# wadx2019/rpo

Measured on AMD Instinct MI355X. Metric: env-steps/sec (whole node), SafeCartpole-v0 (CartSafe-v0) RPODDPG, rollout + one batch-256 constrained policy update per vector step, higher is better.
Workload: dtype f32; 1 GPU; CartSafe-v0 RPODDPG, 4096 vectorised envs per MI355X, scripts/cart_exp.py hyper-parameters, update batch 256 every vector step (reference cadence), replay capacity 20000 per env; envs_per_gpu=4096, global_envs=4096, update_batch=256, hip_graph=True, training_batch_projection=row-wise, rccl_ranks=0, collectives_in_graph=False, graphs_replayed_on_all_ranks=True, graph_capture_fell_back_to_eager=False

## Files before the change

### rpo_amd/csrc/fused.hip

```cpp
#include <stdlib.h>

#include <type_traits>

#include "cartsafe_dev.h"
#include "heads_dev.h"
#include "mlp_bwd.h"
#include "mlp_tile.h"
#include "pendulum_dev.h"
#include "rollout_args.h"
#include "rollout_env.h"

namespace {

using namespace rpo_mlp_dev;
using rpo_cart_dev::ActArgs;
using rpo_cart_dev::CartConsts;
using rpo_cart_dev::cart_explore_project;
using rpo_cart_dev::load_consts;

Mlp to_dev(const rpo_mlp* h) {
    return Mlp{h->Ws, h->bs, h->Wa, h->ba, h->W0, h->b0, h->W1, h->b1, h->W1b, h->b1b, h->S, h->A, h->E, h->H, h->n_out, h->cat, h->head_dim};
}


#ifndef RPO_ROLLOUT_SKIP
#define RPO_ROLLOUT_SKIP 0
#endif

template <class ENV, int EIN, int H, int RT>
__global__ __launch_bounds__(kFwdThreads) void rollout_kernel(RolloutArgs<ENV> p, typename ENV::Consts c) {
    typedef TileLds<EIN, RT, 8, 8> Lds;
    __shared__ Lds lds;
    constexpr int kInS = Lds::kS;
    constexpr int kLanes = rpo_mlp_dev::kRows * RT;
    constexpr int kStats = 10;
    const int row0 = blockIdx.x * kLanes;
    const int tid = threadIdx.x;
    const int n = p.step.n;
    const long long t = p.step.ctrl ? p.step.ctrl[RPO_CTRL_T] : 0;
    RpoEpisode ep{0, 0.0f, 0u};
    if (tid < kLanes && row0 + tid < n) ep = ENV::episode(p.step, row0 + tid);
    ENV::stage_obs(p.step, row0, kLanes, lds.in_s, kInS);
    float draw = 0.0f;
    const bool philox_noise = !p.gauss && p.act.noise_mode == RPO_NOISE_PHILOX;
    if (!(RPO_ROLLOUT_SKIP & 8) && tid < kLanes && row0 + tid < n && (p.gauss || philox_noise)) {
        const rpo_u4 u = p.gauss ? rpo_philox(p.act.seed, p.act.env_id_base + (uint32_t)(row0 + tid), (uint32_t)t, RPO_STREAM_POLICY,
                                              (uint32_t)p.step.ctrl[RPO_CTRL_UPDATES])
                                 : rpo_philox(p.act.seed, p.act.env_id_base + (uint32_t)(row0 + tid), (uint32_t)t, RPO_STREAM_ACT);
        draw = rpo_normal(u.x, u.y);
    }
    if (RPO_ROLLOUT_SKIP & 1) {
        if (tid < 2 * kLanes) lds.out[tid] = 0.25f;
        __syncthreads();
    } else {
        mlp_tile_forward<EIN, H, RT, Lds>(p.actor, lds, row0, n, nullptr, nullptr, p.gauss ? 0 : 1, p.scale, p.base);
    }

    float st[kStats];
#pragma unroll
    for (int k = 0; k < kStats; ++k) st[k] = 0.0f;
    float iters_f = 0.0f;
    const int i = row0 + tid;
    if (tid < kLanes && i < n) {
        const float eps_t = fmaxf(p.act.eps_end, p.act.eps_start - p.act.eps_decay * (float)t);
        float ap = lds.out[tid * 2];
        if (p.gauss) {
            ap = rpo_head_dev::gauss_head_row(ap, lds.out[tid * 2 + 1], draw, p.scale, p.base, p.act.box_lo, p.act.box_hi, 0, nullptr);
        }
        int k;
        typename ENV::ActArgs act = p.act;
        if (philox_noise) {
            ap = rpo_explore_clip(ap, eps_t, draw, p.act.box_lo, p.act.box_hi);
            act.noise_mode = RPO_NOISE_NONE;
        }
        float2 a;
        if (RPO_ROLLOUT_SKIP & 2) { a = make_float2(ap, 0.5f * ap); k = 0; }
        else a = ENV::project(act, c, lds.in_s + tid * kInS, i, ap, eps_t, t, k);
        iters_f = (float)k;
        reinterpret_cast<float2*>(p.act.action)[i] = a;
        const long long ring_base = p.step.rows ? (t % p.step.cap_steps) * (long long)n : 0;
        if (!(RPO_ROLLOUT_SKIP & 4)) ENV::lane(p.step, c, i, lds.in_s + tid * kInS, a, ep, ring_base, st);
    }
    if (RPO_ROLLOUT_SKIP & 16) return;
    if (p.step.stats && tid < 64) {
        float* srow = rpo_stats_row(p.step.stats, p.step.stats_cap, t);
        const int slot[kStats + 1] = {RPO_STAT_REWARD_SUM, RPO_STAT_EPISODES, RPO_STAT_RETURN_SUM, RPO_STAT_LENGTH_SUM,
                                      RPO_STAT_MAX_INEQ_SUM, RPO_STAT_MAX_EQ_SUM, RPO_STAT_VIOL_COUNT, RPO_STAT_TERMINATED,
                                      RPO_STAT_MAX_INEQ_MAX, RPO_STAT_MAX_EQ_MAX, RPO_STAT_PROJ_ITERS};
        float red[kStats + 1];
#pragma unroll
        for (int k = 0; k < kStats; ++k) red[k] = st[k];
        red[kStats] = iters_f;
        if (kLanes <= 16) rpo_row16_reduce_many(red, 3u << 8);
        else rpo_wave_reduce_many<kStats + 1, 32>(red, 3u << 8);
        rpo_stats_commit(red, 3u << 8, slot, srow);
    }
    if (!p.defer_clock) rpo_step_epilogue(p.step.ctrl, t, p.step.stats, p.step.stats_cap);
}

template <class ENV>
int launch_rollout(const RolloutArgs<ENV>& args, const typename ENV::Consts& c, int n_envs, void* stream) {
    {
        const int sel = rpo_tune(RPO_TUNE_ROLLOUT_WIDE);
        if (sel == 3 || sel == 4 || (sel == 2 && n_envs >= RPO_ROLLOUT_STREAM_FROM)) {
            const int e = rpo_rollout_stream_launch(std::is_same<ENV, CartEnv>::value ? 0 : 1, &args, &c, n_envs, stream);
            if (e >= 0) return e;
        }
    }
    const int wide_sel = rpo_tune(RPO_TUNE_ROLLOUT_WIDE);
    const int E = args.actor.E;
    const bool wide = E == 128 && (wide_sel == 0 || wide_sel == 1 ? wide_sel != 0 : n_envs >= 64 * 192);
    if (E == 128 && wide) {
        hipLaunchKernelGGL((rollout_kernel<ENV, 128, 256, 4>), dim3((n_envs + 63) / 64), dim3(kFwdThreads), 0,
                           (hipStream_t)stream, args, c);
    } else if (E == 128) {
        hipLaunchKernelGGL((rollout_kernel<ENV, 128, 256, 1>), dim3((n_envs + 15) / 16), dim3(kFwdThreads), 0,
                           (hipStream_t)stream, args, c);
    } else if (E == 256) {
        hipLaunchKernelGGL((rollout_kernel<ENV, 256, 256, 1>), dim3((n_envs + 15) / 16), dim3(kFwdThreads), 0,
                           (hipStream_t)stream, args, c);
    } else {
        return RPO_ERR_ARG;
    }
    RPO_LAUNCH_CHECK();
    return 0;
}

int check_actor(const Mlp& actor, int obs_dim, int gauss) {
    if (actor.hd > 1 || actor.S != obs_dim || actor.A != 0 || actor.n_out != (gauss ? 2 : 1) || actor.cat || actor.H != 256 || !actor.Ws ||
        !actor.W0 || !actor.W1 || (gauss && !actor.W1b))
        return RPO_ERR_ARG;
    return 0;
}
// ... 1057 lines not shown
```

### rpo_amd/csrc/mlp_tile.h

```cpp
#pragma once
#include "common.h"

namespace rpo_mlp_dev {

typedef float f32x4 __attribute__((ext_vector_type(4)));

constexpr int kRows = 16;
constexpr int kThreads = 256;
constexpr int kFwdWaves = 8;
constexpr int kFwdThreads = kFwdWaves * 64;
constexpr int kInS = 64, kInA = 48;

struct Mlp {
    const float *Ws, *bs, *Wa, *ba, *W0, *b0, *W1, *b1, *W1b, *b1b;
    int S, A, E, H, n_out, cat;
    int hd;
    int l1_vec;
};
struct MlpGrad {
    float *Ws, *bs, *Wa, *ba, *W0, *b0, *W1, *b1, *W1b, *b1b;
};

__device__ __forceinline__ f32x4 mfma4(float a, float b, f32x4 c) {
    return __builtin_amdgcn_mfma_f32_16x16x4f32(a, b, c, 0, 0, 0);
}

template <int EIN, int RT = 1, int INS = kInS, int INA = kInA>
struct TileLds {
    static constexpr int ROWS = kRows * RT;
    static constexpr int kS = INS, kA = INA;
    __attribute__((aligned(16))) float x1[ROWS * (EIN + 4)];
    float in_s[ROWS * INS];
    float in_a[ROWS * INA];
    float part[kFwdWaves * ROWS * 2];
    float out[ROWS * 2];
};

constexpr int kWideOut = 32;

template <int EIN, int H>
struct TileLdsWide : TileLds<EIN, 1, kInS, kInA> {
    __attribute__((aligned(16))) float hr[kRows * (H + 4)];
    float outw[kRows * kWideOut];
};

template <int EIN, int H, int RT>
struct TileWeights {
    static constexpr int NT = H / (16 * kFwdWaves);
    static constexpr int ITS = EIN / 16;
    static constexpr int PRE_MAX = RT > 1 ? 4 : 16;
    static constexpr int PRE = ITS < PRE_MAX ? ITS : PRE_MAX;
    static constexpr int TPW = EIN / (16 * kFwdWaves);
    float bias;
    float ws0[8], wa0[8];
    float wk[TPW][3];
    float4 wpre[PRE][NT];
    float b0v[NT], w1av[NT], w1bv[NT];
    float b1v;
};

template <int EIN>
__device__ __forceinline__ bool tile_l1_mfma(const Mlp& net) {
    return EIN == 128 && !net.cat && net.S <= 6 && net.A <= 4 && net.S > 0 && !net.l1_vec;
}

#ifndef RPO_TILE_SKIP
#define RPO_TILE_SKIP 0
#endif

template <int EIN, int H, int RT>
__device__ __forceinline__ void tile_load_weights(const Mlp& net, TileWeights<EIN, H, RT>& w) {
    constexpr int ROWS = kRows * RT;
    constexpr int NT = TileWeights<EIN, H, RT>::NT, PRE = TileWeights<EIN, H, RT>::PRE;
    const int tid = threadIdx.x, lane = tid & 63, wave = tid >> 6;
    const int li = lane & 15, lg = lane >> 4;
    if (RPO_TILE_SKIP & 1) {
        w.bias = 0.01f * (float)li;
#pragma unroll
        for (int u = 0; u < 8; ++u) { w.ws0[u] = 0.1f; w.wa0[u] = 0.1f; }
#pragma unroll
        for (int it = 0; it < PRE; ++it)
#pragma unroll
            for (int c = 0; c < NT; ++c) w.wpre[it][c] = make_float4(0.01f, -0.01f, 0.02f, 0.01f * (float)lg);
#pragma unroll
        for (int c = 0; c < NT; ++c) { w.b0v[c] = 0.1f; w.w1av[c] = 0.05f; w.w1bv[c] = 0.0f; }
        w.b1v = 0.0f;
        return;
    }
    if (tile_l1_mfma<EIN>(net)) {
        constexpr int TPW = TileWeights<EIN, H, RT>::TPW;
        const bool add_a = net.A > 0;
        w.bias = 0.0f;
#pragma unroll
        for (int t = 0; t < TPW; ++t) {
            const int e = (wave + t * kFwdWaves) * 16 + li;
            const float* p0 = lg == 0 ? net.bs + e : (lg == 1 ? net.ba + e : net.Ws + e * net.S + (lg - 2));
            const bool live0 = lg == 0 || (lg == 1 ? add_a : lg - 2 < net.S);
            w.wk[t][0] = live0 ? *p0 : 0.0f;
            w.wk[t][1] = 2 + lg < net.S ? net.Ws[e * net.S + 2 + lg] : 0.0f;
            w.wk[t][2] = (add_a && lg < net.A) ? net.Wa[e * net.A + lg] : 0.0f;
        }
    } else {
        const int e_col = tid % EIN;
        const bool act_part = net.cat && e_col >= net.E;
        const int er = act_part ? e_col - net.E : e_col;
        const bool use_s = !act_part, use_a = net.A > 0 && (act_part || !net.cat);
        w.bias = act_part ? net.ba[er] : (net.bs[er] + ((net.A > 0 && !net.cat) ? net.ba[er] : 0.0f));
#pragma unroll
        for (int u = 0; u < 8; ++u) {
            w.ws0[u] = (use_s && u < net.S) ? net.Ws[er * net.S + u] : 0.0f;
            w.wa0[u] = (use_a && u < net.A) ? net.Wa[er * net.A + u] : 0.0f;
        }
    }
    const int j0 = wave * (H / kFwdWaves);
#pragma unroll
    for (int it = 0; it < PRE; ++it)
#pragma unroll
        for (int c = 0; c < NT; ++c)
            w.wpre[it][c] = *reinterpret_cast<const float4*>(&net.W0[(size_t)(j0 + c * 16 + li) * EIN + it * 16 + lg * 4]);
#pragma unroll
    for (int c = 0; c < NT; ++c) {
        w.b0v[c] = net.b0[j0 + c * 16 + li];
        w.w1av[c] = net.hd > 1 ? 0.0f : net.W1[j0 + c * 16 + li];
        w.w1bv[c] = (net.n_out > 1 && net.hd <= 1) ? net.W1b[j0 + c * 16 + li] : 0.0f;
    }
    w.b1v = (net.hd <= 1 && tid < ROWS * net.n_out) ? (((tid % net.n_out) == 0) ? net.b1[0] : net.b1b[0]) : 0.0f;
}

template <int EIN, int H, int RT, class LDS, bool WIDE = false>
__device__ __forceinline__ void tile_compute(const Mlp& net, const TileWeights<EIN, H, RT>& w, LDS& lds, int row0, int n,
                                             float* x0_save, float* h1_save, int out_mode, float scale, float base) {
    constexpr int kInS = LDS::kS, kInA = LDS::kA;
    constexpr int ROWS = kRows * RT;
    constexpr int LDX = EIN + 4;
    constexpr int GROUPS = kFwdThreads / EIN;
    constexpr int RPT = ROWS / GROUPS;
    static_assert(kFwdThreads % EIN == 0 && ROWS % GROUPS == 0, "layer-1 thread mapping");
    constexpr int NT = TileWeights<EIN, H, RT>::NT, ITS = TileWeights<EIN, H, RT>::ITS, PRE = TileWeights<EIN, H, RT>::PRE;
    float* x1 = lds.x1;
    const float* in_s = lds.in_s;
    const float* in_a = lds.in_a;
    float* part = lds.part;
    const int tid = threadIdx.x, lane = tid & 63, wave = tid >> 6;
    const int li = lane & 15, lg = lane >> 4;
    const int e_col = tid % EIN, r_lo = (tid / EIN) * RPT;
    const bool act_part = net.cat && e_col >= net.E;
    const int er = act_part ? e_col - net.E : e_col;
    const bool use_s = !act_part, use_a = net.A > 0 && (act_part || !net.cat);
    const int j0 = wave * (H / kFwdWaves);
    float acc1[RPT];
#pragma unroll
    for (int r = 0; r < RPT; ++r) acc1[r] = w.bias;
    __syncthreads();
    const bool l1_mfma = tile_l1_mfma<EIN>(net);
    if (l1_mfma) {
        constexpr int TPW = TileWeights<EIN, H, RT>::TPW;
        const bool x0_vec = (reinterpret_cast<uintptr_t>(x0_save) & 15u) == 0;
#pragma unroll
        for (int rt = 0; rt < RT; ++rt) {
            const int row = rt * kRows + li;
            const float b0 = lg < 2 ? 1.0f : (lg - 2 < net.S ? in_s[row * kInS + lg - 2] : 0.0f);
            const float b1 = 2 + lg < net.S ? in_s[row * kInS + 2 + lg] : 0.0f;
            const float b2 = (net.A > 0 && lg < net.A) ? in_a[row * kInA + lg] : 0.0f;
#pragma unroll
            for (int t = 0; t < TPW; ++t) {
                f32x4 c = f32x4{0.0f, 0.0f, 0.0f, 0.0f};
                if (!(RPO_TILE_SKIP & 2)) {
                    c = mfma4(w.wk[t][0], b0, c);
                    c = mfma4(w.wk[t][1], b1, c);
                    c = mfma4(w.wk[t][2], b2, c);
                }
                const int e0 = (wave + t * kFwdWaves) * 16 + 4 * lg;
                if (x0_save && row0 + row < n) {
                    float* dst = x0_save + (size_t)(row0 + row) * EIN + e0;
                    if (x0_vec) *reinterpret_cast<f32x4*>(dst) = c;
                    else { dst[0] = c[0]; dst[1] = c[1]; dst[2] = c[2]; dst[3] = c[3]; }
                }
                *reinterpret_cast<f32x4*>(&x1[row * LDX + e0]) =
                    f32x4{fmaxf(c[0], 0.0f), fmaxf(c[1], 0.0f), fmaxf(c[2], 0.0f), fmaxf(c[3], 0.0f)};
            }
        }
    }

    if (!l1_mfma && use_s && !(RPO_TILE_SKIP & 2)) {
        for (int i0 = 0; i0 < net.S; i0 += 8) {
            float wv[8];
#pragma unroll
            for (int u = 0; u < 8; ++u) wv[u] = (i0 == 0) ? w.ws0[u] : ((i0 + u < net.S) ? net.Ws[er * net.S + i0 + u] : 0.0f);
#pragma unroll
            for (int u = 0; u < 8; ++u) {
                if (i0 + u < net.S) {
#pragma unroll
                    for (int r = 0; r < RPT; ++r) acc1[r] = fmaf(in_s[(r_lo + r) * kInS + i0 + u], wv[u], acc1[r]);
                }
            }
        }
    }
    if (!l1_mfma && use_a && !(RPO_TILE_SKIP & 2)) {
        for (int i0 = 0; i0 < net.A; i0 += 8) {
            float wv[8];
#pragma unroll
            for (int u = 0; u < 8; ++u) wv[u] = (i0 == 0) ? w.wa0[u] : ((i0 + u < net.A) ? net.Wa[er * net.A + i0 + u] : 0.0f);
#pragma unroll
            for (int u = 0; u < 8; ++u) {
                if (i0 + u < net.A) {
#pragma unroll
                    for (int r = 0; r < RPT; ++r) acc1[r] = fmaf(in_a[(r_lo + r) * kInA + i0 + u], wv[u], acc1[r]);
// ... 131 lines not shown
```

### rpo_amd/csrc/nsplit.hip

```cpp
#include <stdlib.h>

#include "cartsafe_dev.h"
#include "heads_dev.h"
#include "mlp_bwd.h"
#include "nsplit_dev.h"
#include "pendulum_dev.h"
#include "rollout_env.h"

namespace {

using namespace rpo_mlp_dev;

Mlp to_dev(const rpo_mlp* h) {
    return Mlp{h->Ws, h->bs, h->Wa, h->ba, h->W0, h->b0, h->W1, h->b1, h->W1b, h->b1b, h->S, h->A, h->E, h->H, h->n_out, h->cat, h->head_dim};
}

bool split_ok(const Mlp& m) {
    return m.E == 128 && m.H == 256 && !m.cat && m.hd <= 1 && m.S <= 6 && m.A <= 4 && m.n_out >= 1 && m.n_out <= 2 && m.Ws && m.W0 &&
           m.W1 && (m.A == 0 || m.Wa) && (m.n_out == 1 || m.W1b);
}

struct NsBlock { int tile, g; };
__device__ __forceinline__ NsBlock ns_block() {
    const int lin = (int)blockIdx.x + (int)gridDim.x * (int)blockIdx.y, T = (int)gridDim.y;
// ... 724 lines not shown
        __syncthreads();
        float s0 = 0.0f, s1 = 0.0f;
        for (int b2 = tid; b2 < B; b2 += kThreads) {
            s0 += dglob[(size_t)b2 * dstride];
            if (two) s1 += dglob[(size_t)b2 * dstride + 1];
        }
        { float ss[2] = {s0, s1}; rpo_wave_reduce_many(ss, 0u); s0 = ss[0]; s1 = ss[1]; }
        float* red = smem + 256;
        if ((tid & 63) == 0) { red[(tid >> 6) * 2] = s0; red[(tid >> 6) * 2 + 1] = s1; }
        __syncthreads();
        if (tid == 0) {
            const float nb1 = cur_b1 + (((red[0] + red[2]) + red[4]) + red[6]);
            gr.b1[0] = nb1;
            gmax = fmaxf(gmax, fabsf(nb1));
            if (two) {
                const float nb1b = cur_b1b + (((red[1] + red[3]) + red[5]) + red[7]);
                gr.b1b[0] = nb1b;
                gmax = fmaxf(gmax, fabsf(nb1b));
            }
        }
    }
    return gmax;
}

__device__ __forceinline__ float ns_weight_role(const Mlp& net, const MlpGrad& gr, const float* h1, const float* x0,
                                                const float* dglob, int dstride, bool two, int B, int w, float* smem) {
    if (w < kW0Tiles) return ns_dw0_tile(net, gr.W0, h1, x0, dglob, dstride, two, B, w, smem);
    return ns_hv_block(net, gr, h1, dglob, dstride, two, B, w - kW0Tiles, smem);
}

constexpr int kBwdASmem = kRows * (256 + 4) + 16 + 4 * 16 * 16;

template <class L>
__device__ __forceinline__ void bwd_a_role(const SplitArgs& p, float* smem, int b, unsigned fused_consumers = 0u,
                                           unsigned fused_need = 0u, unsigned fused_need_critics = 0u) {
    constexpr int EIN = 128, H = 256, LDH = H + 4;
    const int T = (p.B + kRows - 1) / kRows, B = p.B;
    const int tid = threadIdx.x, lane = tid & 63, wave = tid >> 6, li = lane & 15, lg = lane >> 4;
    {
        const int k = b / (T * kNsGroups), rem = b - k * T * kNsGroups, g = rem / T, tile = rem - g * T;
        const int row0 = tile * kRows;
        const Mlp& net = p.critic[k];
        float* dh_s = smem;
        float* dq_s = smem + kRows * LDH;
        float* wpart = dq_s + 16;
        const int jw = wave * (H / 4), e = g * 16 + li;
        float wv[H / 16], hv[kRows];
#pragma unroll
        for (int ks = 0; ks < H / 16; ++ks) wv[ks] = net.W0[(size_t)(jw + ks * 4 + lg) * EIN + e];
        const float w1a = net.W1[tid];
        if (fused_consumers && fused_need_critics)
            ns_tile_wait(p.tile_sync + (T + tile) * kNsSyncStride, fused_need_critics, p.tile_sync + 3 * T * kNsSyncStride, 16);
#pragma unroll
        for (int r = 0; r < kRows; ++r) hv[r] = row0 + r < B ? p.h1[k][(size_t)(row0 + r) * H + tid] : 0.0f;
        const size_t xo = (size_t)(row0 + (tid >> 4)) * EIN + g * 16 + (tid & 15);
        const float x0v = row0 + (tid >> 4) < B ? p.x0[k][xo] : 0.0f;
        if (fused_consumers) {
            ns_tile_wait(p.tile_sync + (T + tile) * kNsSyncStride, fused_need, p.tile_sync + 3 * T * kNsSyncStride);
            ns_tile_passed(p.tile_sync, T, tile, fused_consumers);
        }
        if (tid < 64) {
            float dq = 0.0f, hub = 0.0f;
            if (tid < kRows && row0 + tid < B) {
                dq = ns_td_row<L>(p, k, row0 + tid, &hub);
                if (g == 0) p.dq[k][row0 + tid] = dq;
            }
            if (tid < kRows) dq_s[tid] = dq;
            const float sum = rpo_row16_sum_desc_lane0(hub);
            if (tid == 0 && g == 0) p.loss_partial[k * T + tile] = sum;
        }
        __syncthreads();
#pragma unroll
        for (int r = 0; r < kRows; ++r) dh_s[r * LDH + tid] = (hv[r] > 0.0f) ? dq_s[r] * w1a : 0.0f;
        __syncthreads();
        f32x4 acc = f32x4{0.0f, 0.0f, 0.0f, 0.0f};
#pragma unroll
        for (int ks = 0; ks < H / 16; ++ks) acc = mfma4(dh_s[li * LDH + jw + ks * 4 + lg], wv[ks], acc);
#pragma unroll
        for (int i = 0; i < 4; ++i) wpart[(wave * 16 + lg * 4 + i) * 16 + li] = acc[i];
        __syncthreads();
        {
            const int r = tid >> 4, ee = tid & 15;
            float v = wpart[(0 * 16 + r) * 16 + ee];
            v = wpart[(1 * 16 + r) * 16 + ee] + v;
            v = wpart[(2 * 16 + r) * 16 + ee] + v;
            v = wpart[(3 * 16 + r) * 16 + ee] + v;
            if (row0 + r < B) p.dx0[k][xo] = x0v > 0.0f ? v : 0.0f;
        }
    }
}

template <class L>
__global__ __launch_bounds__(kThreads) void split_critic_bwd_a_kernel(SplitArgs p) {
    __shared__ __attribute__((aligned(16))) float smem[kBwdASmem];
    bwd_a_role<L>(p, smem, blockIdx.x);
}

__device__ __forceinline__ void adam_prepare(int* step_dev, float beta1, float beta2) {
    const int s = step_dev[0] + 1;
    double* cache = reinterpret_cast<double*>(step_dev + 4);
    cache[0] = 1.0 - pow((double)beta1, (double)s);
    cache[1] = sqrt(1.0 - pow((double)beta2, (double)s));
    step_dev[1] = s;
    step_dev[0] = s;
}

__device__ __forceinline__ void bwd_b_bookkeeping(const SplitArgs& p) {
    if (threadIdx.x != 0) return;
    if (p.prep_step) adam_prepare(p.prep_step, p.prep_beta1, p.prep_beta2);
    if (p.clock_out) p.clock_out[0] += 1;
    if (p.updates_out) p.updates_out[RPO_CTRL_UPDATES] += 1;
}

template <class L>
__device__ __forceinline__ void bwd_b_role(const SplitArgs& p, float* smem, int bx, int k, int own_blocks) {
    if ((p.prep_step || p.clock_out || p.updates_out) && bx == own_blocks - 1) {
        if (k == 0) bwd_b_bookkeeping(p);
        return;
    }
    if (bx < kWeightBlocks) {
        gradmax_flush(p.gradmax, ns_weight_role(p.critic[k], p.critic_grad[k], p.h1[k], p.x0[k], p.dq[k], 1, false, p.B, bx, smem));
        return;
    }
    BwdArgs a{};
    a.net = p.critic[k];
    a.g = p.critic_grad[k];
// ... 357 lines not shown
        if (tid < 64) {
            const int r = tid / 3, q = tid - 3 * r;
            const bool mine = tid < 48 && row0 + r < B;
            unsigned long long x = 0;
            for (int spins = 0;; ++spins) {
                bool ok = true;
                if (mine) { x = pm_load(ws + kPmAct + (size_t)(row0 + r) * 3 + q); ok = (x >> 32) == tag0; }
                if (__all(ok)) break;
                if (spins >= kPmSpinMax) { x = 0; __hip_atomic_store(ws + kPmGaveUp, 1ull, __ATOMIC_RELAXED, __HIP_MEMORY_SCOPE_AGENT); break; }
            }
            if (mine) {
                const float v = __uint_as_float((unsigned)x);
                if (q < 2) lds.in_a[r * 8 + q] = v;
                else if (p.twin && g == 0 && k == 0) p.logp[row0 + r] = v;
            }
        }
        PM_STAMP(ws, nb.tile == 0 && g == 0 && k == 0, 50);
        pm_reader_done(ws, tag0, readers);
        ns_hidden<128, 256>(net, w, lds, g, row0, B, p.part_qn[k], nullptr, nullptr, pre);
        ns_tile_arrive(sync + (T + nb.tile) * kNsSyncStride);
        PM_STAMP(ws, nb.tile == 0 && g == 0 && k == 0, 51);
    } else {
        pol_a_role<L>(p, lds, tile, row0, g, sync + nb.tile * kNsSyncStride, (unsigned)kNsGroups);
        ns_tile_passed(sync, T, nb.tile, consumers);
    }
    return true;
}

static_assert(kPmSmem + 256 + 16 + 4 * kRows * 4 <= kFrontSmem, "projection role fits");

template <class L>
__global__ __launch_bounds__(kThreads) void split_critic_pfront_kernel(SplitArgs p, CartConsts c, int pol, unsigned long long* ws,
                                                                      int store_mode) {
    __shared__ __attribute__((aligned(16))) float smem[kFrontSmem];
    pfront_role<L>(p, c, smem, pol, ws, store_mode);
}

template <class L>
__global__ __launch_bounds__(kThreads) void split_critic_pfront_ride_kernel(SplitArgs p, CartConsts c, RideArgs<typename L::Env> r,
                                                                           unsigned long long* ws, int store_mode) {
    __shared__ __attribute__((aligned(16))) float smem[kFrontSmem];
    if (pfront_role<L>(p, c, smem, 0, ws, store_mode)) return;
    const NsBlock nb = ns_block();
    const int own = 2 + 3 * (p.twin ? 2 : 1);
    ride_forward_pair<typename L::Env>(r, reinterpret_cast<NsLds<128>*>(smem), ((int)blockIdx.z - own) * (int)gridDim.y + nb.tile, nb.g);
}

template <class ENV>
__device__ __forceinline__ void pol_b_role(const SplitArgs& p, const CartConsts& c, NsLds<128>& lds, float4* tile, int tile_i, int g,
                                           int k, unsigned* wait_word = nullptr, unsigned wait_need = 0u) {
    typedef typename ENV::L L;
    const int row0 = tile_i * kRows, tid = threadIdx.x, B = p.B;
    const Mlp& net = p.critic[k];
    NsWeights<128> w;
    ns_load_weights<128, 256>(net, g, w);
    ns_load_tile<L>(p, tile, row0);
    __syncthreads();
    ns_stage<L>(lds, reinterpret_cast<const float*>(tile), false, false);
    __syncthreads();
    float pre[kRows];
    if (wait_word) {
        ns_layer1_state<128>(net, w, lds, pre);
        const int T = (B + kRows - 1) / kRows;
        ns_tile_wait(wait_word, wait_need, p.tile_sync + 3 * T * kNsSyncStride);
    }
    const bool writer = g == 0 && k == 0;
    float vals[7] = {0, 0, 0, 0, 0, 0, 0};
    if (tid < kRows) {
        const int i = row0 + tid;
        float2 act = make_float2(0.0f, 0.0f);
        if (i < B) {
            const long long t = p.ctrl[RPO_CTRL_T];
            const float inv_b = 1.0f / (float)B;
            float e;
            if (p.eps_in) {
                e = p.eps_in[i];
            } else {
                const rpo_u4 u = rpo_philox(p.noise_seed, p.noise_id_base + (uint32_t)i, (uint32_t)t + p.noise_salt,
                                            RPO_STREAM_POLICY, (uint32_t)p.ctrl[RPO_CTRL_UPDATES]);
                e = rpo_normal(u.x, u.y);
            }
            float ap, logp = 0.0f, rm = 0.0f, rl = 0.0f, ap_det = 0.0f;
            if (p.twin) {
                rm = ns_head(pol_part(p), B, i, 0, p.actor.b1[0]);
                rl = ns_head(pol_part(p), B, i, 1, p.actor.b1b[0]);
                ap = rpo_head_dev::gauss_head_row(rm, rl, e, p.scale, p.base, p.box_lo, p.box_hi, 0, &logp);
            } else {
                const float v = ns_head(pol_part(p), B, i, 0, p.actor.b1[0]);
                ap_det = p.scale * tanhf(v) + p.base;
                const float eps_t = fmaxf(p.eps_end, p.eps_start - p.eps_decay * (float)t);
                ap = explore_clip(ap_det, eps_t, e, p.box_lo, p.box_hi);
            }
            act = ENV::complete(c, lds.in_s + tid * 8, i, ap, t);
            if (writer) {
                if (p.twin) {
                    reinterpret_cast<float2*>(p.raw)[i] = make_float2(rm, rl);
                    p.logp[i] = logp;
                } else {
                    p.ap_det[i] = ap_det;
                }
                p.noise_out[i] = e;
                reinterpret_cast<float2*>(p.actions)[i] = act;
                float dist[6];
                float2 gg;
                vals[0] = ENV::lagr(c, act.x, act.y, p.nu, inv_b, dist, gg);
#pragma unroll
                for (int j = 0; j < 6; ++j) vals[1 + j] = dist[j];
                reinterpret_cast<float2*>(p.g_act)[i] = gg;
            }
        }
        lds.in_a[tid * 8] = act.x;
        lds.in_a[tid * 8 + 1] = act.y;
    }
    if (writer && tid < 64) {
#pragma unroll
        for (int q = 0; q < 7; ++q) {
            const float sum = rpo_row16_sum_desc_lane0(vals[q]);
            if (tid == 0) p.lag_partial[tile_i * 8 + q] = sum;
        }
    }
    ns_hidden<128, 256>(net, w, lds, g, row0, B, p.part_q[k], p.x0[k], p.h1[k], wait_word ? pre : nullptr);
}

template <class ENV>
__global__ __launch_bounds__(kNsThreads) void split_policy_b_kernel(SplitArgs p, CartConsts c) {
    __shared__ NsLds<128> lds;
    __shared__ __attribute__((aligned(16))) float4 tile[kRows * ENV::L::CH];
    const NsBlock nb = ns_block();
    pol_b_role<ENV>(p, c, lds, tile, nb.tile, nb.g, blockIdx.z);
}

__device__ __forceinline__ float ns_policy_dq(const SplitArgs& p, int k, int i, float* term) {
    const float inv_b = 1.0f / (float)p.B;
    const float q1 = ns_head(p.part_q[0], p.B, i, 0, p.critic[0].b1[0]);
    if (!p.twin) {
        *term = q1;
        return -inv_b;
    }
    const float q2 = ns_head(p.part_q[1], p.B, i, 0, p.critic[1].b1[0]);
    const float w1 = (q1 < q2 ? 1.0f : 0.0f) + (q1 == q2 ? 0.5f : 0.0f);
    *term = p.alpha * p.logp[i] - fminf(q1, q2);
    return k == 0 ? w1 * -inv_b : (1.0f - w1) * -inv_b;
}

__device__ __forceinline__ void pol_c_role(const SplitArgs& p, float* smem, int b, unsigned fused_consumers = 0u,
                                           unsigned fused_need = 0u) {
    constexpr int EIN = 128, H = 256, LDH = H + 4;
    float* dh_s = smem;
    float* dq_s = smem + kRows * LDH;
    float* wpart = dq_s + 16;
    const int T = (p.B + kRows - 1) / kRows, B = p.B;
    const int tid = threadIdx.x, lane = tid & 63, wave = tid >> 6, li = lane & 15, lg = lane >> 4;
    const int k = b / (T * kNsGroups), rem = b - k * T * kNsGroups, g = rem / T, tile = rem - g * T;
    const int row0 = tile * kRows;
    const Mlp& net = p.critic[k];
    const int jw = wave * (H / 4), e = g * 16 + li;
    float wv[H / 16], hv[kRows];
#pragma unroll
    for (int ks = 0; ks < H / 16; ++ks) wv[ks] = net.W0[(size_t)(jw + ks * 4 + lg) * EIN + e];
    const float w1a = net.W1[tid];
    const float2 wa2 = *reinterpret_cast<const float2*>(&net.Wa[(g * 16 + (tid & 15)) * 2]);
    if (fused_consumers) {
        ns_tile_wait(p.tile_sync + (T + tile) * kNsSyncStride, fused_need, p.tile_sync + 3 * T * kNsSyncStride);
        ns_tile_passed(p.tile_sync, T, tile, fused_consumers);
    }
#pragma unroll
    for (int r = 0; r < kRows; ++r) hv[r] = row0 + r < B ? p.h1[k][(size_t)(row0 + r) * H + tid] : 0.0f;
    const size_t xo = (size_t)(row0 + (tid >> 4)) * EIN + g * 16 + (tid & 15);
    const float x0v = row0 + (tid >> 4) < B ? p.x0[k][xo] : 0.0f;
    if (tid < 64) {
        float dq = 0.0f, term = 0.0f;
        if (tid < kRows && row0 + tid < B) dq = ns_policy_dq(p, k, row0 + tid, &term);
        if (tid < kRows) dq_s[tid] = dq;
        const float sum = rpo_row16_sum_desc_lane0(term);
        if (tid == 0 && g == 0 && k == 0) p.lag_partial[tile * 8 + 7] = sum;
    }
    __syncthreads();
#pragma unroll
    for (int r = 0; r < kRows; ++r) dh_s[r * LDH + tid] = (hv[r] > 0.0f) ? dq_s[r] * w1a : 0.0f;
    __syncthreads();
    f32x4 acc = f32x4{0.0f, 0.0f, 0.0f, 0.0f};
#pragma unroll
    for (int ks = 0; ks < H / 16; ++ks) acc = mfma4(dh_s[li * LDH + jw + ks * 4 + lg], wv[ks], acc);
#pragma unroll
    for (int i = 0; i < 4; ++i) wpart[(wave * 16 + lg * 4 + i) * 16 + li] = acc[i];
    __syncthreads();
    {
        const int r = tid >> 4, ee = tid & 15;
        float v = wpart[(0 * 16 + r) * 16 + ee];
        v = wpart[(1 * 16 + r) * 16 + ee] + v;
        v = wpart[(2 * 16 + r) * 16 + ee] + v;
        v = wpart[(3 * 16 + r) * 16 + ee] + v;
        const bool live = row0 + r < B;
        v = (live && x0v > 0.0f) ? v : 0.0f;
        if (live) p.dx0[k][xo] = v;
        float d0 = v * wa2.x, d1 = v * wa2.y;
        d0 = rpo_row16_sum_lane0(d0); d1 = rpo_row16_sum_lane0(d1);
        if (ee == 0 && live)
            reinterpret_cast<float2*>(p.da_part)[((size_t)k * kNsGroups + g) * B + row0 + r] = make_float2(d0, d1);
    }
}

__global__ __launch_bounds__(kThreads) void split_policy_c_kernel(SplitArgs p) {
    __shared__ __attribute__((aligned(16))) float smem[kBwdASmem];
    pol_c_role(p, smem, blockIdx.x);
}


template <class ENV>
__device__ __forceinline__ float2 ns_policy_dout(const SplitArgs& p, const CartConsts& c, int i) {
    typedef typename ENV::L L;
    const int K = p.twin ? 2 : 1;
    float da0 = 0.0f, da1 = 0.0f;
    for (int k = 0; k < K; ++k) {
        float s0 = 0.0f, s1 = 0.0f;
#pragma unroll
        for (int g = 0; g < kNsGroups; ++g) {
            const float2 d = reinterpret_cast<const float2*>(p.da_part)[((size_t)k * kNsGroups + g) * p.B + i];
            s0 += d.x; s1 += d.y;
        }
        da0 = k == 0 ? s0 : da0 + s0;
        da1 = k == 0 ? s1 : da1 + s1;
    }
    const float2 gg = reinterpret_cast<const float2*>(p.g_act)[i];
    da0 += gg.x; da1 += gg.y;
    const float dap = ENV::complete_bwd(c, p.batch_out + (size_t)i * L::ROW, da0, da1);
    if (p.twin) {
        const float2 r = reinterpret_cast<const float2*>(p.raw)[i];
        return rpo_head_dev::gauss_head_bwd_row(r.x, r.y, p.noise_out[i], dap, p.alpha / (float)p.B, p.scale, p.base, p.box_lo,
                                                p.box_hi);
    }
    const float t = (float)p.ctrl[RPO_CTRL_T];
    const float eps_t = fmaxf(p.eps_end, p.eps_start - p.eps_decay * t);
    return make_float2(rpo_head_dev::tanh_box_bwd_row(dap, p.ap_det[i], p.noise_out[i], 1, eps_t, p.box_lo, p.box_hi, p.scale,
                                                      p.base), 0.0f);
}

template <class ENV>
__device__ __forceinline__ void pol_d_role(const SplitArgs& p, const CartConsts& c, float* smem, int b, unsigned fused_consumers = 0u,
                                           unsigned fused_need_a = 0u, unsigned fused_need_c = 0u) {
    constexpr int EIN = 128, H = 256, LDH = H + 4;
    const int B = p.B;
    const int tid = threadIdx.x, lane = tid & 63, wave = tid >> 6, li = lane & 15, lg = lane >> 4;
    const Mlp& net = p.actor;
    {
        const int T = (B + kRows - 1) / kRows, g = b / T, tile = b - g * T, row0 = tile * kRows;
        float* dh_s = smem;
        float* do_s = smem + kRows * LDH;
        float* wpart = do_s + 32;
        const int jw = wave * (H / 4), e = g * 16 + li;
        float wv[H / 16], hv[kRows];
#pragma unroll
        for (int ks = 0; ks < H / 16; ++ks) wv[ks] = net.W0[(size_t)(jw + ks * 4 + lg) * EIN + e];
        const float w1a = net.W1[tid], w1b = net.n_out > 1 ? net.W1b[tid] : 0.0f;
        unsigned* gave_up = p.tile_sync ? p.tile_sync + 3 * T * kNsSyncStride : nullptr;
        if (fused_consumers && fused_need_a) ns_tile_wait(p.tile_sync + tile * kNsSyncStride, fused_need_a, gave_up);
#pragma unroll
        for (int r = 0; r < kRows; ++r) hv[r] = row0 + r < B ? p.h1_a[(size_t)(row0 + r) * H + tid] : 0.0f;
        const size_t xo = (size_t)(row0 + (tid >> 4)) * EIN + g * 16 + (tid & 15);
        const bool xlive = row0 + (tid >> 4) < B;
        const float x0v = xlive ? p.x0_a[xo] : 0.0f;
        if (fused_consumers) {
            ns_tile_wait(p.tile_sync + tile * kNsSyncStride, fused_need_c, gave_up, 16);
            ns_tile_passed(p.tile_sync, T, tile, fused_consumers);
        }
        float cdx = 0.0f;
        if (xlive && p.shared_embedding) cdx = p.twin ? p.dx0[0][xo] + p.dx0[1][xo] : p.dx0[0][xo];
        if (tid < kRows) {
            float2 d = make_float2(0.0f, 0.0f);
            if (row0 + tid < B) {
                d = ns_policy_dout<ENV>(p, c, row0 + tid);
                if (g == 0) reinterpret_cast<float2*>(p.dout)[row0 + tid] = d;
            }
            do_s[tid * 2] = d.x; do_s[tid * 2 + 1] = d.y;
        }
        __syncthreads();
#pragma unroll
        for (int r = 0; r < kRows; ++r)
            dh_s[r * LDH + tid] = (hv[r] > 0.0f) ? fmaf(do_s[r * 2 + 1], w1b, do_s[r * 2] * w1a) : 0.0f;
        __syncthreads();
        f32x4 acc = f32x4{0.0f, 0.0f, 0.0f, 0.0f};
#pragma unroll
        for (int ks = 0; ks < H / 16; ++ks) acc = mfma4(dh_s[li * LDH + jw + ks * 4 + lg], wv[ks], acc);
#pragma unroll
        for (int i = 0; i < 4; ++i) wpart[(wave * 16 + lg * 4 + i) * 16 + li] = acc[i];
        __syncthreads();
        {
            const int r = tid >> 4, ee = tid & 15;
            float v = wpart[(0 * 16 + r) * 16 + ee];
            v = wpart[(1 * 16 + r) * 16 + ee] + v;
            v = wpart[(2 * 16 + r) * 16 + ee] + v;
            v = wpart[(3 * 16 + r) * 16 + ee] + v;
            if (xlive) {
                v = x0v > 0.0f ? v : 0.0f;
                if (p.shared_embedding) v += cdx;
                p.dx0_a[xo] = v;
            }
        }
    }
}

constexpr int kPolDSmem = kRows * (256 + 4) + 32 + 4 * 16 * 16;

template <class ENV>
__global__ __launch_bounds__(kThreads) void split_policy_d_kernel(SplitArgs p, CartConsts c) {
    __shared__ __attribute__((aligned(16))) float smem[kPolDSmem];
    pol_d_role<ENV>(p, c, smem, blockIdx.x);
}

constexpr int kPolFrontSmem = kPolDSmem > kFrontSmem ? kPolDSmem : kFrontSmem;

template <class ENV>
__global__ __launch_bounds__(kThreads) void split_policy_front_kernel(SplitArgs p, CartConsts c, int with_a) {
    typedef typename ENV::L L;
    __shared__ __attribute__((aligned(16))) float smem[kPolFrontSmem];
    const int K = p.twin ? 2 : 1, T = (int)gridDim.y, z = (int)blockIdx.z;
    const int lin = (int)blockIdx.x + (int)gridDim.x * (int)blockIdx.y;
    const unsigned consumers = (unsigned)(kNsGroups * (K * (1 + with_a) + 1));
    if (z == with_a + 2 * K) {
        pol_d_role<ENV>(p, c, smem, lin, consumers, with_a ? (unsigned)kNsGroups : 0u, (unsigned)(kNsGroups * K));
        return;
    }
    if (z >= with_a + K) {
        pol_c_role(p, smem, (z - with_a - K) * T * kNsGroups + lin, consumers, (unsigned)(kNsGroups * K));
        ns_tile_arrive(p.tile_sync + (lin % T) * kNsSyncStride, 1u << 16);
        return;
    }
    if (threadIdx.x >= kNsThreads) return;
    NsLds<128>& lds = *reinterpret_cast<NsLds<128>*>(smem);
    float4* tile = reinterpret_cast<float4*>(reinterpret_cast<char*>(smem) + sizeof(NsLds<128>));
    const NsBlock nb = ns_block();
    unsigned* sync = p.tile_sync;
// ... 609 lines not shown
```

### rpo_amd/csrc/nsplit_dev.h

```cpp
#pragma once
#include "mlp_tile.h"

namespace rpo_mlp_dev {

constexpr int kNsThreads = 128;
constexpr int kNsGroups = 8;

template <int EIN>
struct NsLds {
    __attribute__((aligned(16))) float x1[kRows * (EIN + 4)];
    float in_s[kRows * 8];
    float in_a[kRows * 8];
    float xch[2 * 4 * 64];
};

template <int EIN>
struct NsWeights {
    float wk[4][3];
    float4 w0[EIN / 16];
    float b0v, w1av, w1bv;
};

__device__ __forceinline__ float ns_l1_state_w(const Mlp& net, int e, int u) {
    const float* ptr = u == 0 ? net.bs + e : (u == 1 ? net.ba + e : net.Ws + e * net.S + (u - 2));
// ... 67 lines not shown
        if (act) {
            c = mfma4(w.wk[t][2], b2, c);
        }
        const int e0 = 64 * wave + 16 * t + 4 * lg;
        if (x0_save && g == 0 && row0 + li < n) {
            float* dst = x0_save + (size_t)(row0 + li) * EIN + e0;
            if (x0_vec) *reinterpret_cast<f32x4*>(dst) = c;
            else { dst[0] = c[0]; dst[1] = c[1]; dst[2] = c[2]; dst[3] = c[3]; }
        }
        *reinterpret_cast<f32x4*>(&lds.x1[li * LDX + e0]) =
            f32x4{fmaxf(c[0], 0.0f), fmaxf(c[1], 0.0f), fmaxf(c[2], 0.0f), fmaxf(c[3], 0.0f)};
    }
    __syncthreads();
    f32x4 acc = f32x4{0.0f, 0.0f, 0.0f, 0.0f};
#pragma unroll
    for (int it = 0; it < EIN / 16; ++it) {
        const float4 a4 = *reinterpret_cast<const float4*>(&lds.x1[li * LDX + it * 16 + lg * 4]);
        acc = mfma4(a4.x, w.w0[it].x, acc);
        acc = mfma4(a4.y, w.w0[it].y, acc);
        acc = mfma4(a4.z, w.w0[it].z, acc);
        acc = mfma4(a4.w, w.w0[it].w, acc);
    }
    const int col = g * 32 + wave * 16 + li;
    float hr[4];
#pragma unroll
    for (int i = 0; i < 4; ++i) {
        const float h = acc[i] + w.b0v;
        const int row = row0 + lg * 4 + i;
        if (h1_save && row < n) h1_save[(size_t)row * H + col] = h;
        hr[i] = fmaxf(h, 0.0f);
    }
    if (wave == 0) {
#pragma unroll
        for (int i = 0; i < 4; ++i) {
            lds.xch[(0 * 4 + i) * 64 + lane] = fmaf(hr[i], w.w1av, 0.0f);
            lds.xch[(1 * 4 + i) * 64 + lane] = fmaf(hr[i], w.w1bv, 0.0f);
        }
    }
    __syncthreads();
    if (wave == 1) {
#pragma unroll
        for (int o = 0; o < 2; ++o)
#pragma unroll
            for (int i = 0; i < 4; ++i) {
                float v = fmaf(hr[i], o == 0 ? w.w1av : w.w1bv, lds.xch[(o * 4 + i) * 64 + lane]);
                v = rpo_row16_sum_lane0(v);
                const int row = row0 + lg * 4 + i;
                if (li == 0 && row < n && o < net.n_out) part[((size_t)g * n + row) * 2 + o] = v;
                if (hp) hp[o][i] = v;
            }
    }
}

__device__ __forceinline__ float ns_head(const float* part, int n, int row, int o, float bias) {
    float v = bias;
#pragma unroll
    for (int g = 0; g < kNsGroups; ++g) v += part[((size_t)g * n + row) * 2 + o];
    return v;
}

}
```

### rpo_amd/csrc/rollout_env.h

```cpp
#pragma once
#include "cartsafe_dev.h"
#include "pendulum_dev.h"

namespace {

struct CartEnv {
    typedef rpo_cart_dev::StepArgs StepArgs;
    typedef rpo_cart_dev::ActArgs ActArgs;
    typedef rpo_cart_dev::CartConsts Consts;
    static constexpr int OBS = 6;
    __device__ static __forceinline__ void stage_obs(const StepArgs& p, int row0, int rows, float* in_s, int stride, int tid_in = -1) {
        const int tid = tid_in < 0 ? (int)threadIdx.x : tid_in;
        if (tid < rows * 6) {
            const int r = tid / 6, i = tid - r * 6;
            in_s[r * stride + i] = (row0 + r < p.n) ? p.state[(size_t)(row0 + r) * 6 + i] : 0.0f;
        }
    }
    __device__ static __forceinline__ void lane_obs(const StepArgs& p, int i, float (&o)[8]) {
#pragma unroll
        for (int q = 0; q < 6; ++q) o[q] = p.state[(size_t)i * 6 + q];
        o[6] = o[7] = 0.0f;
    }
    __device__ static __forceinline__ float2 project(const ActArgs& a, const Consts& c, const float* obs, int i, float ap,
                                                     float eps_t, long long t, int& k) {
        return rpo_cart_dev::cart_explore_project(a, c, i, ap, eps_t, t, k);
    }
    __device__ static __forceinline__ float2 project_budget(const ActArgs& a, const Consts& c, const float* obs, int i, float ap,
                                                            int max_steps, float corr_lr, int& k) {
        return rpo_cart_dev::cart_explore_project(a, c, i, ap, 0.0f, 0, k, RpoBudgetOfLane{max_steps, corr_lr});
    }
    __device__ static __forceinline__ RpoEpisode episode(const StepArgs& p, int i) {
        return rpo_load_episode(p.ep_len, p.ep_ret, p.ep_count, i);
    }
    __device__ static __forceinline__ void lane(const StepArgs& p, const Consts& c, int i, const float* obs, float2 a,
                                                const RpoEpisode& ep, long long ring_base,
                                                float (&st)[rpo_cart_dev::kStepStats], bool full_line = false) {
        float s[6], ns[6];
        float4 row[6];
#pragma unroll
        for (int q = 0; q < 6; ++q) s[q] = obs[q];
        rpo_cart_dev::cart_lane(p, c, i, s, a, ep, ns, row, st);
        if (p.rows) {
            float4* gr = reinterpret_cast<float4*>(p.rows + (size_t)(ring_base + i) * RPO_CART_RING);
#pragma unroll
            for (int q = 0; q < 6; ++q) gr[q] = row[q];
            if (full_line) {
#pragma unroll
                for (int q = 6; q < RPO_CART_RING / 4; ++q) gr[q] = make_float4(0.0f, 0.0f, 0.0f, 0.0f);
            }
        }
        rpo_cart_dev::store_state(p.state + (size_t)i * 6, ns);
    }
    __device__ __host__ static __forceinline__ const float* obs_rows(const StepArgs& p) { return p.state; }
};

struct PendEnv {
    typedef rpo_pend_dev::StepArgs StepArgs;
    typedef rpo_pend_dev::ActArgs ActArgs;
    struct Consts { int unused; };
    static constexpr int OBS = 5;
    __device__ static __forceinline__ void stage_obs(const StepArgs& p, int row0, int rows, float* in_s, int stride, int tid_in = -1) {
        const int tid = tid_in < 0 ? (int)threadIdx.x : tid_in;
        if (tid < rows) {
            float4 s = make_float4(0.0f, 0.0f, 1.0f, 0.0f);
            if (row0 + tid < p.n) s = reinterpret_cast<const float4*>(p.internal)[row0 + tid];
            float sn, cs;
            sincosf(s.x, &sn, &cs);
            float* o = in_s + tid * stride;
            o[0] = cs; o[1] = sn; o[2] = s.y; o[3] = s.z; o[4] = s.w;
        }
    }
    __device__ static __forceinline__ void lane_obs(const StepArgs& p, int i, float (&o)[8]) {
        const float4 s = reinterpret_cast<const float4*>(p.internal)[i];
        float sn, cs;
        sincosf(s.x, &sn, &cs);
        o[0] = cs; o[1] = sn; o[2] = s.y; o[3] = s.z; o[4] = s.w;
        o[5] = o[6] = o[7] = 0.0f;
    }
    __device__ static __forceinline__ float2 project(const ActArgs& a, const Consts&, const float* obs, int i, float ap,
                                                     float eps_t, long long t, int& k) {
        return rpo_pend_dev::pend_explore_project(a, obs, i, ap, eps_t, t, k);
    }
    __device__ static __forceinline__ float2 project_budget(const ActArgs& a, const Consts&, const float* obs, int i, float ap,
                                                            int max_steps, float corr_lr, int& k) {
        return rpo_pend_dev::pend_explore_project(a, obs, i, ap, 0.0f, 0, k, RpoBudgetOfLane{max_steps, corr_lr});
    }
    __device__ static __forceinline__ RpoEpisode episode(const StepArgs& p, int i) {
        return rpo_load_episode(p.ep_len, p.ep_ret, p.ep_count, i);
    }
    __device__ static __forceinline__ void lane(const StepArgs& p, const Consts&, int i, const float* obs, float2 a,
                                                const RpoEpisode& ep, long long ring_base,
                                                float (&st)[rpo_pend_dev::kStepStats], bool full_line = false) {
        const float4 s = reinterpret_cast<const float4*>(p.internal)[i];
        float ns[4], ncs, nsn;
        float4 row[4];
        rpo_pend_dev::pend_lane(p, i, s, a, ep, ns, ncs, nsn, row, st);
        if (p.rows) {
            float4* gr = reinterpret_cast<float4*>(p.rows + (size_t)(ring_base + i) * RPO_PEND_RING);
#pragma unroll
            for (int q = 0; q < 4; ++q) gr[q] = row[q];
        }
        reinterpret_cast<float4*>(p.internal)[i] = make_float4(ns[0], ns[1], ns[2], ns[3]);
        if (p.obs) rpo_pend_dev::store_obs(p.obs + (size_t)i * 5, ncs, nsn, ns[1], ns[2], ns[3]);
    }
    __device__ __host__ static __forceinline__ const float* obs_rows(const StepArgs& p) { return p.obs; }
};

}
```

Before: 101.7 million env-steps/s.

## Overlap observation and weight loads with compute in rollout and nsplit backward kernels

The rollout kernel now issues the observation global load first into registers, loads the actor tile weights, and only then commits the observations to LDS before computing, so the two memory latencies overlap. In the nsplit backward kernels, hidden and input loads become unconditional by clamping the row index, with the row mask moved to the use site. Empty asm barriers keep these loads in flight across syncs. Policy clock values are hoisted out of the per-row branch. This costs extra registers and possibly occupancy, and relies on the clamped loads staying in bounds.

```diff
diff --git a/rpo_amd/csrc/fused.hip b/rpo_amd/csrc/fused.hip
--- a/rpo_amd/csrc/fused.hip
+++ b/rpo_amd/csrc/fused.hip
@@ -38,9 +38,9 @@
     const int tid = threadIdx.x;
     const int n = p.step.n;
     const long long t = p.step.ctrl ? p.step.ctrl[RPO_CTRL_T] : 0;
+    typename ENV::ObsReg obs_reg = ENV::obs_request(p.step, row0, kLanes);
     RpoEpisode ep{0, 0.0f, 0u};
     if (tid < kLanes && row0 + tid < n) ep = ENV::episode(p.step, row0 + tid);
-    ENV::stage_obs(p.step, row0, kLanes, lds.in_s, kInS);
     float draw = 0.0f;
     const bool philox_noise = !p.gauss && p.act.noise_mode == RPO_NOISE_PHILOX;
     if (!(RPO_ROLLOUT_SKIP & 8) && tid < kLanes && row0 + tid < n && (p.gauss || philox_noise)) {
@@ -53,7 +53,10 @@
         if (tid < 2 * kLanes) lds.out[tid] = 0.25f;
         __syncthreads();
     } else {
-        mlp_tile_forward<EIN, H, RT, Lds>(p.actor, lds, row0, n, nullptr, nullptr, p.gauss ? 0 : 1, p.scale, p.base);
+        TileWeights<EIN, H, RT> w;
+        tile_load_weights<EIN, H, RT>(p.actor, w);
+        ENV::obs_commit(obs_reg, kLanes, lds.in_s, kInS);
+        tile_compute<EIN, H, RT, Lds>(p.actor, w, lds, row0, n, nullptr, nullptr, p.gauss ? 0 : 1, p.scale, p.base);
     }
 
     float st[kStats];
@@ -79,6 +82,7 @@
         iters_f = (float)k;
         reinterpret_cast<float2*>(p.act.action)[i] = a;
         const long long ring_base = p.step.rows ? (t % p.step.cap_steps) * (long long)n : 0;
+        asm volatile("" : "+v"(ep.len), "+v"(ep.ret), "+v"(ep.count));
         if (!(RPO_ROLLOUT_SKIP & 4)) ENV::lane(p.step, c, i, lds.in_s + tid * kInS, a, ep, ring_base, st);
     }
     if (RPO_ROLLOUT_SKIP & 16) return;
diff --git a/rpo_amd/csrc/mlp_tile.h b/rpo_amd/csrc/mlp_tile.h
--- a/rpo_amd/csrc/mlp_tile.h
+++ b/rpo_amd/csrc/mlp_tile.h
@@ -51,7 +51,7 @@
     static constexpr int PRE_MAX = RT > 1 ? 4 : 16;
     static constexpr int PRE = ITS < PRE_MAX ? ITS : PRE_MAX;
     static constexpr int TPW = EIN / (16 * kFwdWaves);
-    float bias;
+    float bias, bias_a;
     float ws0[8], wa0[8];
     float wk[TPW][3];
     float4 wpre[PRE][NT];
@@ -75,7 +75,7 @@
     const int tid = threadIdx.x, lane = tid & 63, wave = tid >> 6;
     const int li = lane & 15, lg = lane >> 4;
     if (RPO_TILE_SKIP & 1) {
-        w.bias = 0.01f * (float)li;
+        w.bias = 0.01f * (float)li; w.bias_a = 0.0f;
 #pragma unroll
         for (int u = 0; u < 8; ++u) { w.ws0[u] = 0.1f; w.wa0[u] = 0.1f; }
 #pragma unroll
@@ -90,22 +90,25 @@
     if (tile_l1_mfma<EIN>(net)) {
         constexpr int TPW = TileWeights<EIN, H, RT>::TPW;
         const bool add_a = net.A > 0;
-        w.bias = 0.0f;
 #pragma unroll
         for (int t = 0; t < TPW; ++t) {
             const int e = (wave + t * kFwdWaves) * 16 + li;
             const float* p0 = lg == 0 ? net.bs + e : (lg == 1 ? net.ba + e : net.Ws + e * net.S + (lg - 2));
             const bool live0 = lg == 0 || (lg == 1 ? add_a : lg - 2 < net.S);
+            int m1 = e * net.S, ma = e * net.A;
+            asm volatile("" : "+v"(m1), "+v"(ma));
+            const int i1 = m1 + 2 + lg, ia = ma + lg;
             w.wk[t][0] = live0 ? *p0 : 0.0f;
-            w.wk[t][1] = 2 + lg < net.S ? net.Ws[e * net.S + 2 + lg] : 0.0f;
-            w.wk[t][2] = (add_a && lg < net.A) ? net.Wa[e * net.A + lg] : 0.0f;
+            w.wk[t][1] = 2 + lg < net.S ? net.Ws[i1] : 0.0f;
+            w.wk[t][2] = (add_a && lg < net.A) ? net.Wa[ia] : 0.0f;
         }
     } else {
         const int e_col = tid % EIN;
         const bool act_part = net.cat && e_col >= net.E;
         const int er = act_part ? e_col - net.E : e_col;
         const bool use_s = !act_part, use_a = net.A > 0 && (act_part || !net.cat);
-        w.bias = act_part ? net.ba[er] : (net.bs[er] + ((net.A > 0 && !net.cat) ? net.ba[er] : 0.0f));
+        w.bias = act_part ? net.ba[er] : net.bs[er];
+        w.bias_a = (!act_part && net.A > 0 && !net.cat) ? net.ba[er] : 0.0f;
 #pragma unroll
         for (int u = 0; u < 8; ++u) {
             w.ws0[u] = (use_s && u < net.S) ? net.Ws[er * net.S + u] : 0.0f;
@@ -148,11 +151,11 @@
     const int er = act_part ? e_col - net.E : e_col;
     const bool use_s = !act_part, use_a = net.A > 0 && (act_part || !net.cat);
     const int j0 = wave * (H / kFwdWaves);
+    const bool l1_mfma = tile_l1_mfma<EIN>(net);
     float acc1[RPT];
 #pragma unroll
-    for (int r = 0; r < RPT; ++r) acc1[r] = w.bias;
+    for (int r = 0; r < RPT; ++r) acc1[r] = l1_mfma ? 0.0f : (act_part ? w.bias : w.bias + w.bias_a);
     __syncthreads();
-    const bool l1_mfma = tile_l1_mfma<EIN>(net);
     if (l1_mfma) {
         constexpr int TPW = TileWeights<EIN, H, RT>::TPW;
         const bool x0_vec = (reinterpret_cast<uintptr_t>(x0_save) & 15u) == 0;
diff --git a/rpo_amd/csrc/nsplit.hip b/rpo_amd/csrc/nsplit.hip
--- a/rpo_amd/csrc/nsplit.hip
+++ b/rpo_amd/csrc/nsplit.hip
@@ -800,9 +800,9 @@
         if (fused_consumers && fused_need_critics)
             ns_tile_wait(p.tile_sync + (T + tile) * kNsSyncStride, fused_need_critics, p.tile_sync + 3 * T * kNsSyncStride, 16);
 #pragma unroll
-        for (int r = 0; r < kRows; ++r) hv[r] = row0 + r < B ? p.h1[k][(size_t)(row0 + r) * H + tid] : 0.0f;
+        for (int r = 0; r < kRows; ++r) hv[r] = p.h1[k][(size_t)ns_clamp_row(row0 + r, B) * H + tid];
         const size_t xo = (size_t)(row0 + (tid >> 4)) * EIN + g * 16 + (tid & 15);
-        const float x0v = row0 + (tid >> 4) < B ? p.x0[k][xo] : 0.0f;
+        const float x0v = p.x0[k][ns_clamp_xo(xo, row0 + (tid >> 4), B, EIN)];
         if (fused_consumers) {
             ns_tile_wait(p.tile_sync + (T + tile) * kNsSyncStride, fused_need, p.tile_sync + 3 * T * kNsSyncStride);
             ns_tile_passed(p.tile_sync, T, tile, fused_consumers);
@@ -818,8 +818,9 @@
             if (tid == 0 && g == 0) p.loss_partial[k * T + tile] = sum;
         }
         __syncthreads();
-#pragma unroll
-        for (int r = 0; r < kRows; ++r) dh_s[r * LDH + tid] = (hv[r] > 0.0f) ? dq_s[r] * w1a : 0.0f;
+        ns_keep_in_flight(hv);
+#pragma unroll
+        for (int r = 0; r < kRows; ++r) dh_s[r * LDH + tid] = (row0 + r < B && hv[r] > 0.0f) ? dq_s[r] * w1a : 0.0f;
         __syncthreads();
         f32x4 acc = f32x4{0.0f, 0.0f, 0.0f, 0.0f};
 #pragma unroll
@@ -1283,6 +1284,7 @@
     typedef typename ENV::L L;
     const int row0 = tile_i * kRows, tid = threadIdx.x, B = p.B;
     const Mlp& net = p.critic[k];
+    const long long clk_t = p.ctrl[RPO_CTRL_T], clk_updates = p.ctrl[RPO_CTRL_UPDATES];
     NsWeights<128> w;
     ns_load_weights<128, 256>(net, g, w);
     ns_load_tile<L>(p, tile, row0);
@@ -1301,14 +1303,14 @@
         const int i = row0 + tid;
         float2 act = make_float2(0.0f, 0.0f);
         if (i < B) {
-            const long long t = p.ctrl[RPO_CTRL_T];
+            const long long t = clk_t;
             const float inv_b = 1.0f / (float)B;
             float e;
             if (p.eps_in) {
                 e = p.eps_in[i];
             } else {
                 const rpo_u4 u = rpo_philox(p.noise_seed, p.noise_id_base + (uint32_t)i, (uint32_t)t + p.noise_salt,
-                                            RPO_STREAM_POLICY, (uint32_t)p.ctrl[RPO_CTRL_UPDATES]);
+                                            RPO_STREAM_POLICY, (uint32_t)clk_updates);
                 e = rpo_normal(u.x, u.y);
             }
             float ap, logp = 0.0f, rm = 0.0f, rl = 0.0f, ap_det = 0.0f;
@@ -1396,9 +1398,9 @@
         ns_tile_passed(p.tile_sync, T, tile, fused_consumers);
     }
 #pragma unroll
-    for (int r = 0; r < kRows; ++r) hv[r] = row0 + r < B ? p.h1[k][(size_t)(row0 + r) * H + tid] : 0.0f;
+    for (int r = 0; r < kRows; ++r) hv[r] = p.h1[k][(size_t)ns_clamp_row(row0 + r, B) * H + tid];
     const size_t xo = (size_t)(row0 + (tid >> 4)) * EIN + g * 16 + (tid & 15);
-    const float x0v = row0 + (tid >> 4) < B ? p.x0[k][xo] : 0.0f;
+    const float x0v = p.x0[k][ns_clamp_xo(xo, row0 + (tid >> 4), B, EIN)];
     if (tid < 64) {
         float dq = 0.0f, term = 0.0f;
         if (tid < kRows && row0 + tid < B) dq = ns_policy_dq(p, k, row0 + tid, &term);
@@ -1407,8 +1409,9 @@
         if (tid == 0 && g == 0 && k == 0) p.lag_partial[tile * 8 + 7] = sum;
     }
     __syncthreads();
-#pragma unroll
-    for (int r = 0; r < kRows; ++r) dh_s[r * LDH + tid] = (hv[r] > 0.0f) ? dq_s[r] * w1a : 0.0f;
+    ns_keep_in_flight(hv);
+#pragma unroll
+    for (int r = 0; r < kRows; ++r) dh_s[r * LDH + tid] = (row0 + r < B && hv[r] > 0.0f) ? dq_s[r] * w1a : 0.0f;
     __syncthreads();
     f32x4 acc = f32x4{0.0f, 0.0f, 0.0f, 0.0f};
 #pragma unroll
@@ -1487,10 +1490,10 @@
         unsigned* gave_up = p.tile_sync ? p.tile_sync + 3 * T * kNsSyncStride : nullptr;
         if (fused_consumers && fused_need_a) ns_tile_wait(p.tile_sync + tile * kNsSyncStride, fused_need_a, gave_up);
 #pragma unroll
-        for (int r = 0; r < kRows; ++r) hv[r] = row0 + r < B ? p.h1_a[(size_t)(row0 + r) * H + tid] : 0.0f;
+        for (int r = 0; r < kRows; ++r) hv[r] = p.h1_a[(size_t)ns_clamp_row(row0 + r, B) * H + tid];
         const size_t xo = (size_t)(row0 + (tid >> 4)) * EIN + g * 16 + (tid & 15);
         const bool xlive = row0 + (tid >> 4) < B;
-        const float x0v = xlive ? p.x0_a[xo] : 0.0f;
+        const float x0v = p.x0_a[ns_clamp_xo(xo, row0 + (tid >> 4), B, EIN)];
         if (fused_consumers) {
             ns_tile_wait(p.tile_sync + tile * kNsSyncStride, fused_need_c, gave_up, 16);
             ns_tile_passed(p.tile_sync, T, tile, fused_consumers);
@@ -1506,9 +1509,10 @@
             do_s[tid * 2] = d.x; do_s[tid * 2 + 1] = d.y;
         }
         __syncthreads();
+        ns_keep_in_flight(hv);
 #pragma unroll
         for (int r = 0; r < kRows; ++r)
-            dh_s[r * LDH + tid] = (hv[r] > 0.0f) ? fmaf(do_s[r * 2 + 1], w1b, do_s[r * 2] * w1a) : 0.0f;
+            dh_s[r * LDH + tid] = (row0 + r < B && hv[r] > 0.0f) ? fmaf(do_s[r * 2 + 1], w1b, do_s[r * 2] * w1a) : 0.0f;
         __syncthreads();
         f32x4 acc = f32x4{0.0f, 0.0f, 0.0f, 0.0f};
 #pragma unroll
diff --git a/rpo_amd/csrc/nsplit_dev.h b/rpo_amd/csrc/nsplit_dev.h
--- a/rpo_amd/csrc/nsplit_dev.h
+++ b/rpo_amd/csrc/nsplit_dev.h
@@ -143,6 +143,16 @@
     }
 }
 
+__device__ __forceinline__ int ns_clamp_row(int row, int n) { return row < n ? row : n - 1; }
+__device__ __forceinline__ size_t ns_clamp_xo(size_t xo, int row, int n, int width) {
+    return row < n ? xo : xo - (size_t)(row - (n - 1)) * (size_t)width;
+}
+__device__ __forceinline__ void ns_keep_in_flight(float (&v)[kRows]) {
+    static_assert(kRows == 16, "operand lists below");
+    asm volatile("" : "+v"(v[8]), "+v"(v[9]), "+v"(v[10]), "+v"(v[11]), "+v"(v[12]), "+v"(v[13]), "+v"(v[14]), "+v"(v[15]));
+    asm volatile("" : "+v"(v[0]), "+v"(v[1]), "+v"(v[2]), "+v"(v[3]), "+v"(v[4]), "+v"(v[5]), "+v"(v[6]), "+v"(v[7]));
+}
+
 __device__ __forceinline__ float ns_head(const float* part, int n, int row, int o, float bias) {
     float v = bias;
 #pragma unroll
diff --git a/rpo_amd/csrc/rollout_env.h b/rpo_amd/csrc/rollout_env.h
--- a/rpo_amd/csrc/rollout_env.h
+++ b/rpo_amd/csrc/rollout_env.h
@@ -15,6 +15,15 @@
             const int r = tid / 6, i = tid - r * 6;
             in_s[r * stride + i] = (row0 + r < p.n) ? p.state[(size_t)(row0 + r) * 6 + i] : 0.0f;
         }
+    }
+    typedef float ObsReg;
+    __device__ static __forceinline__ ObsReg obs_request(const StepArgs& p, int row0, int rows) {
+        const int tid = threadIdx.x, r = tid / 6;
+        return (tid < rows * 6 && row0 + r < p.n) ? p.state[(size_t)row0 * 6 + tid] : 0.0f;
+    }
+    __device__ static __forceinline__ void obs_commit(ObsReg v, int rows, float* in_s, int stride) {
+        const int tid = threadIdx.x, r = tid / 6, i = tid - r * 6;
+        if (tid < rows * 6) in_s[r * stride + i] = v;
     }
     __device__ static __forceinline__ void lane_obs(const StepArgs& p, int i, float (&o)[8]) {
 #pragma unroll
@@ -70,6 +79,22 @@
             o[0] = cs; o[1] = sn; o[2] = s.y; o[3] = s.z; o[4] = s.w;
         }
     }
+    typedef float4 ObsReg;
+    __device__ static __forceinline__ ObsReg obs_request(const StepArgs& p, int row0, int rows) {
+        const int tid = threadIdx.x;
+        float4 s = make_float4(0.0f, 0.0f, 1.0f, 0.0f);
+        if (tid < rows && row0 + tid < p.n) s = reinterpret_cast<const float4*>(p.internal)[row0 + tid];
+        return s;
+    }
+    __device__ static __forceinline__ void obs_commit(ObsReg s, int rows, float* in_s, int stride) {
+        const int tid = threadIdx.x;
+        if (tid < rows) {
+            float sn, cs;
+            sincosf(s.x, &sn, &cs);
+            float* o = in_s + tid * stride;
+            o[0] = cs; o[1] = sn; o[2] = s.y; o[3] = s.z; o[4] = s.w;
+        }
+    }
     __device__ static __forceinline__ void lane_obs(const StepArgs& p, int i, float (&o)[8]) {
         const float4 s = reinterpret_cast<const float4*>(p.internal)[i];
         float sn, cs;
```

Measured after the change: 102.7 million env-steps/s (median of 6 runs). +1.0%, better.
